# celliern/triflow

Measured on AMD Instinct MI355X. Metric: implicit time-steps/s, 1e6-node 3-var system (member-steps/s over all GPUs), higher is better.
Workload: dtype f64; 1 GPU; BASELINE config 3: M3_film, N=1000000 nodes, periodic, fixed dt=0.001, ROS2; members_per_gpu=1, parallelism=ensemble members sharded by rank, no data-path collective

## Files before the change

__graft_entry__.py:

```python
import os
import sys

ROOT = os.path.dirname(os.path.abspath(__file__))
if ROOT not in sys.path:
    sys.path.insert(0, ROOT)

PREBUILT = ["M1_advdiff", "M2_diff", "M3_film", "M5_stiff"]
PREBUILT_DENSE = ["M3_film", "M5_stiff"]


def build():
    from triflow_amd import compilers, workloads
    from triflow_amd.model import Model
    compilers.build_runtime_library()
    for name in PREBUILT:
        model = Model(*workloads.model_args(name), hold_compilation=True)
        for seg in (4, 8):
            compilers.build_code_object(model, 0, seg=seg)
    saved = os.environ.get("TRIFLOW_BLOCK_MASK")
    os.environ["TRIFLOW_BLOCK_MASK"] = "0"
    try:
        for name in PREBUILT_DENSE:
            model = Model(*workloads.model_args(name), hold_compilation=True)
            compilers.build_code_object(model, 0, seg=4)
    finally:
        if saved is None:
            del os.environ["TRIFLOW_BLOCK_MASK"]
        else:
            os.environ["TRIFLOW_BLOCK_MASK"] = saved
    import triflow_amd


def smoke():
    import numpy as np
    from triflow_amd import Model, schemes, workloads
    from oracle import numpy_path as ora
    name, fd, pars, dt, _ = workloads.config_inputs(3, 4096)
    model = Model(*workloads.model_args(name))
    ref = Model(*workloads.model_args(name), compiler=ora.numpy_compiler)
    F = model.F(model.fields_template(**fd), pars)
    Fo = ref.F(ref.fields_template(**fd), pars)
    assert np.array_equal(F, Fo), "F differs from the oracle"
    J = model.J(model.fields_template(**fd), pars)
    Jo = ref.J(ref.fields_template(**fd), pars)
    assert abs(J - Jo).max() <= 4 * np.spacing(abs(Jo).max()), "J differs from the oracle"
    _, new = schemes.ROS2(model)(0.0, model.fields_template(**fd), dt, pars)
    _, new_o = ora.ROS2(ref)(0.0, ref.fields_template(**fd), dt, pars)
    err = np.abs(new.uflat - new_o.uflat).max() / np.abs(new_o.uflat).max()
    assert err < 1e-9, "ROS2 step differs from the oracle: %g" % err
    print("smoke ok: F bit-exact, J <= 4 ulp, ROS2 step rel err %.1e on %s (N=4096)" % (err, name))


if __name__ == "__main__":
    build()
```

triflow_amd/compilers.py:

```python

import fcntl
import json
import logging
import os
import re
import shutil
import subprocess
import threading
import warnings

import numpy as np
import scipy.sparse as sps

from . import codegen
from ._capi import DeviceModel, DeviceSolver, Library

log = logging.getLogger(__name__)
log.addHandler(logging.NullHandler())

PKG_DIR = os.path.dirname(os.path.abspath(__file__))
CSRC = os.path.join(PKG_DIR, "csrc")
LIB_PATH = os.path.join(PKG_DIR, "lib", "libtriflow_hip.so")
CACHE_DIR = os.path.join(PKG_DIR, "_cache")
GPU_ARCH = "gfx950"
HIPCC_FLAGS = [*os.environ.get("TRIFLOW_HIPCC_OPT", "-O3").split(), "-std=c++17",
               "-ffp-contract=off", "--offload-arch=" + GPU_ARCH,
               *os.environ.get("TRIFLOW_HIPCC_EXTRA", "").split()]

RUNTIME_SOURCES = ("tf_rt_plan.cpp", "tf_rt_io.cpp", "tf_rt_steps.cpp", "tf_rt_diag.cpp",
                   "tf_solver_sweeps.cpp", "tf_solver_linear.cpp", "tf_rt_probe.cpp", "tf_rt_record.cpp",
                   "tf_rt_stat.cpp", "tf_rt_spectrum.cpp", "tf_rt_extrema.cpp")
_SKELETON = ("tf_args.h", "tf_math.h", "tf_kernels.h", "tf_crs.h", "tf_coop_hip.h", "tf_cr2_hip.h", "tf_cr3_hip.h",
             "tf_node.h", "tf_probe.h", "tf_record.h", "tf_stat.h", "tf_spectrum.h", "tf_extrema.h",
             "tf_entry_hip.h")
_TU_HEAD = ('#include <hip/hip_runtime.h>\n'
            '#define TF_DEVICE __device__ __forceinline__\n'
            '%s'
            '#include "tf_math.h"\n')

_TU_TAIL = '#include "tf_kernels.h"\n#include "tf_entry_hip.h"\n'


def _hipcc():
    exe = shutil.which("hipcc") or "/opt/rocm/bin/hipcc"
    if not os.path.exists(exe):
        raise RuntimeError("hipcc not found: the HIP compiler plugin needs the ROCm toolchain")
    return exe


def _skeleton_stamp():
    parts = []
    for name in _SKELETON:
        with open(os.path.join(CSRC, name), "rb") as f:
            parts.append(f.read())
    return codegen.source_hash(*parts)


def build_runtime_library(force=False):
    srcs = [os.path.join(CSRC, n) for n in RUNTIME_SOURCES] + [os.path.join(CSRC, "tf_backend_hip.cpp")]
    deps = srcs + [os.path.join(CSRC, n) for n in ("tf_args.h", "tf_backend.h", "tf_solver.h")] + \
        [os.path.join(os.path.dirname(PKG_DIR), "include", "triflow_hip.h")]
    if not force and os.path.exists(LIB_PATH) and \
            all(os.path.getmtime(LIB_PATH) >= os.path.getmtime(d) for d in deps):
        return LIB_PATH
    os.makedirs(os.path.dirname(LIB_PATH), exist_ok=True)
    cmd = [_hipcc(), "-O2", "-std=c++17", "-fPIC", "-shared", "--offload-arch=" + GPU_ARCH,
           "-I", CSRC, *srcs, "-lpthread", "-o", LIB_PATH + ".tmp"]
    res = subprocess.run(cmd, capture_output=True, text=True)
    if res.returncode != 0:
        raise RuntimeError("building libtriflow_hip.so failed:\n" + res.stderr[-4000:])
    os.replace(LIB_PATH + ".tmp", LIB_PATH)
    return LIB_PATH


def _parse_resource_usage(stderr):
    usage, name = {}, None
    for line in stderr.splitlines():
        m = re.search(r"Function Name: (\S+)", line)
        if m:
            name = m.group(1)
            usage[name] = {}
            continue
        for key, pat in (("VGPRs", r" VGPRs: (\d+)"), ("SGPRs", r" SGPRs: (\d+)"),
                         ("ScratchSize", r"ScratchSize \[bytes/lane\]: (\d+)"),
                         ("Occupancy", r"Occupancy \[waves/SIMD\]: (\d+)")):
            m = re.search(pat, line)
            if m and name:
                usage[name][key] = int(m.group(1))
    return usage


def resource_usage(hsaco_path):
    with open(hsaco_path[:-len(".hsaco")] + ".json") as f:
        return json.load(f)["kernels"]


def _compile_code_object(model, source, tag, hsaco, observer=None):
    global BUILD_COUNT
    BUILD_COUNT += 1
    hip = os.path.join(CACHE_DIR, "model_%s.hip" % tag)
    hip_tmp = hip + ".%d.tmp" % os.getpid()
    with open(hip_tmp, "w") as f:
        f.write(source)
    os.replace(hip_tmp, hip)
    tmp = hsaco + ".%d.tmp" % os.getpid()
    log.info("hipcc: compiling stencil + solver kernels for %s", model._diff_eqs)

    def compile_with(flags, out):
        cmd = [_hipcc(), *flags, "-I", CSRC, "--genco", "--no-gpu-bundle-output",
               "-Rpass-analysis=kernel-resource-usage", "-o", out, hip]
        res = subprocess.run(cmd, capture_output=True, text=True)
        if res.returncode != 0:
            raise RuntimeError("hipcc failed on the generated kernels (%s):\n%s"
                               % (hip, res.stderr[-4000:]))
        return _parse_resource_usage(res.stderr)

    flags = list(HIPCC_FLAGS)
    usage = compile_with(flags, tmp)
    spilled = sorted(k for k, u in usage.items() if u.get("ScratchSize", 0) > 0)
    if observer:
        spilled = [k for k in spilled if k.startswith("tfk_" + observer)]
        if spilled:
            os.remove(tmp)
            raise codegen.UnsupportedExpression(
                "the %s kernels (%s) need more registers than a wavefront has: "
                "use fewer or simpler %ss" % (observer, ", ".join(spilled),
                                               {"stat": "statistic"}.get(observer, observer)))
    alt_flags, alt_usage = None, None
    alt = hsaco[:-len(".hsaco")] + ".alt.hsaco"
    if spilled and "-O1" not in flags and "-O0" not in flags \
            and os.environ.get("TRIFLOW_ALLOW_SCRATCH") != "1":
        _warn_wide(model, spilled)
        alt_flags = ["-O1"] + [f for f in flags if not f.startswith("-O")]
        if os.environ.get("TRIFLOW_SPILL_GATE") == "object":
            flags, alt_flags = alt_flags, None
            usage = compile_with(flags, tmp)
        else:
            alt_usage = compile_with(alt_flags, alt + ".%d.tmp" % os.getpid())
            os.replace(alt + ".%d.tmp" % os.getpid(), alt)
    meta = os.path.join(CACHE_DIR, "model_%s.json" % tag)
    with open(meta + ".%d.tmp" % os.getpid(), "w") as f:
        json.dump(dict(equations=list(model._diff_eqs), flags=flags, kernels=usage,
                       alt_flags=alt_flags, alt_kernels=spilled if alt_flags else [],
                       alt_usage={k: alt_usage[k] for k in spilled} if alt_usage else {},
                       skeleton=_skeleton_stamp(), hipcc=hipcc_version()), f, indent=1)
    os.replace(meta + ".%d.tmp" % os.getpid(), meta)
    os.replace(tmp, hsaco)
    evict_stale_cache()


_warned_wide = set()


def _warn_wide(model, kernels):
    key = tuple(str(e) for e in model._diff_eqs)
    if key in _warned_wide:
        return
    _warned_wide.add(key)
    warnings.warn("triflow_amd: %d kernel(s) of the model %s need more registers than a wavefront has "
                  "(%s spill to scratch): those kernels are built at -O1 and run slower than the "
                  "narrow-model path (DESIGN.md, solver limits)"
                  % (len(kernels), list(key), ", ".join(kernels)), RuntimeWarning, stacklevel=4)


def alternate_of(hsaco_path):
    try:
        with open(hsaco_path[:-len(".hsaco")] + ".json") as f:
            meta = json.load(f)
    except (OSError, ValueError):
        return None, []
    alt = hsaco_path[:-len(".hsaco")] + ".alt.hsaco"
    kernels = meta.get("alt_kernels") or []
    return (alt, kernels) if kernels and os.path.exists(alt) else (None, [])


def _build_locked(model, source, tag, hsaco, observer=None):
    if os.path.exists(hsaco):
        return
    lock_path = hsaco + ".lock"
    try:
        with open(lock_path, "w") as lock:
            try:
                fcntl.flock(lock, fcntl.LOCK_EX)
            except OSError:
                pass
            try:
                if not os.path.exists(hsaco):
                    _compile_code_object(model, source, tag, hsaco, observer)
            finally:
                try:
                    fcntl.flock(lock, fcntl.LOCK_UN)
                except OSError:
                    pass
    finally:
        for leftover in [lock_path] + [os.path.join(CACHE_DIR, n) for n in os.listdir(CACHE_DIR)
                                        if n.endswith(".%d.tmp" % os.getpid())]:
            try:
                os.remove(leftover)
            except OSError:
                pass


def code_object_source(model, parvec_mask=0, seg=8, sweep_block=256):
    body, spec = codegen.lower_model(model, parvec_mask=parvec_mask, seg=seg,
                                     sweep_block=sweep_block)
    source = _TU_HEAD % "" + body + _TU_TAIL
    tag = codegen.source_hash(source, _skeleton_stamp(), " ".join(HIPCC_FLAGS), hipcc_version(), os.environ.get("TRIFLOW_SPILL_GATE", "kernel"), "elf")
    return source, tag, spec


def build_code_object(model, parvec_mask=0, seg=None, sweep_block=None):
    seg = seg or int(os.environ.get("TRIFLOW_SWEEP_SEG", "8"))
    sweep_block = sweep_block or int(os.environ.get("TRIFLOW_SWEEP_BLOCK", "256"))
    source, tag, spec = code_object_source(model, parvec_mask, seg, sweep_block)
    os.makedirs(CACHE_DIR, exist_ok=True)
    hsaco = os.path.join(CACHE_DIR, "model_%s.hsaco" % tag)
    _build_locked(model, source, tag, hsaco)
    return hsaco, spec


def build_observer_code_object(model, block, kind, parvec_mask=0, seg=8, sweep_block=256):
    if kind not in ("probe", "record", "stat", "spectrum", "extrema"):
        raise ValueError("unknown kind of observer %r" % (kind,))
    body, _ = codegen.lower_model(model, parvec_mask=parvec_mask, seg=seg, sweep_block=sweep_block)
    source = _TU_HEAD % "" + body + block + _TU_TAIL
    tag = codegen.source_hash(source, _skeleton_stamp(), " ".join(HIPCC_FLAGS), hipcc_version(), kind, "elf")
    os.makedirs(CACHE_DIR, exist_ok=True)
    hsaco = os.path.join(CACHE_DIR, "model_%s.hsaco" % tag)
    _build_locked(model, source, tag, hsaco, observer=kind)
    return hsaco


_hipcc_version = None
BUILD_COUNT = 0


def hipcc_version():
    global _hipcc_version
    if _hipcc_version is None:
        try:
            res = subprocess.run([_hipcc(), "--version"], capture_output=True, text=True)
            lines = [ln.strip() for ln in res.stdout.splitlines() if ln.strip()]
            _hipcc_version = " / ".join(ln for ln in lines if "version" in ln.lower())[:200] or "unknown"
        except OSError:
            _hipcc_version = "unknown"
    return _hipcc_version


def evict_stale_cache(keep=()):
    if not os.path.isdir(CACHE_DIR):
        return 0
    stamp, ver, removed = _skeleton_stamp(), hipcc_version(), 0
    for name in os.listdir(CACHE_DIR):
        if not (name.startswith("model_") and name.endswith(".json")):
            continue
        base = os.path.join(CACHE_DIR, name[:-len(".json")])
        try:
            with open(base + ".json") as f:
                meta = json.load(f)
        except (OSError, ValueError):
            continue
        if meta.get("skeleton") == stamp and meta.get("hipcc") == ver:
            continue
        if os.path.basename(base) in keep:
            continue
        for ext in (".hsaco", ".alt.hsaco", ".hip", ".json"):
            try:
                os.remove(base + ext)
                removed += 1
            except OSError:
                pass
    return removed


class HipBackend:

    _lib = None
    _lock = threading.Lock()

    def library(self):
        with HipBackend._lock:
            if HipBackend._lib is None:
                HipBackend._lib = Library(LIB_PATH)
            return HipBackend._lib

    def load(self, model, parvec_mask, device=-1, seg=None):
        hsaco, spec = build_code_object(model, parvec_mask, seg=seg)
        lib = self.library()
        is_dev, ndev = lib.runtime_info()
        if ndev < 1:
            raise RuntimeError("no HIP device visible: the triflow_amd compute path needs "
                               "an MI355X (gfx950); there is no CPU fallback")
        if device >= 0:
            lib.set_device(device)
        with open(hsaco, "rb") as f:
            code = f.read()
        alt, alt_kernels = alternate_of(hsaco)
        alt_code = None
        if alt_kernels:
            _warn_wide(model, alt_kernels)
        if alt:
            with open(alt, "rb") as f:
                alt_code = f.read()
        return DeviceModel(lib, spec, code, alt_code, alt_kernels)


_default_backend = HipBackend()


class CscPattern:

    def __init__(self, nvar, mp, sparse_indices, N, periodic):
        k = np.asarray(sparse_indices, dtype=np.int64)
        eq, slot = k % nvar, k // nvar
        var, off = slot % nvar, slot // nvar - mp
        node = np.arange(N, dtype=np.int64)[:, None]
        neigh = node + off[None, :]
        neigh = neigh % N if periodic else np.clip(neigh, 0, N - 1)
        rows = (node * nvar + eq[None, :]).ravel()
        cols = (neigh * nvar + var[None, :]).ravel()
        n = N * nvar
        key = cols * n + rows
        uniq, inverse = np.unique(key, return_inverse=True)
        self.shape = (n, n)
        self.slot = inverse
        self.nslots = uniq.size
        self.indices = (uniq % n).astype(np.int32 if n < 2 ** 31 else np.int64)
        ucols = uniq // n
        self.indptr = np.searchsorted(ucols, np.arange(n + 1)).astype(self.indices.dtype)
        order = np.argsort(inverse, kind="stable")
        first = np.ones(order.size, dtype=bool)
        first[1:] = inverse[order[1:]] != inverse[order[:-1]]
        self.extra_src = order[~first]
        self.extra_slot = inverse[self.extra_src]
        self.gather = np.concatenate([order[first], self.extra_src]).astype(np.int32) \
            if key.size < 2 ** 31 else None

    def assemble(self, values):
        data = np.bincount(self.slot, weights=np.asarray(values).ravel(),
                           minlength=self.nslots)
        return sps.csc_matrix((data, self.indices, self.indptr), shape=self.shape)

    def from_gathered(self, gathered):
        data = gathered[:self.nslots]
        if self.extra_src.size:
            data = data.copy()
            np.add.at(data, self.extra_slot, gathered[self.nslots:])
        return sps.csc_matrix((data, self.indices, self.indptr), shape=self.shape)


class CompiledModel:

    def __init__(self, model, backend=None):
        self.model = model
        self.backend = backend or _default_backend
        self.nvar = model._nvar
        self.fields = list(model._dep_vars) + list(model._help_funcs)
        self.nh = len(model._help_funcs)
        self.pars = list(model._pars)
        self.mp = max((model._window_range - 1) // 2, 1)
        self.real_mp = (model._window_range - 1) // 2
        self._device_models = {}
        self._solvers = {}
        self._patterns = {}
        codegen.lower_model(model)

    @staticmethod
    def sweep_segment(total_nodes):
        if "TRIFLOW_SWEEP_SEG" in os.environ:
            return int(os.environ["TRIFLOW_SWEEP_SEG"])
        return 4 if total_nodes <= 2_000_000 else 8

    def device_model(self, parvec_mask=0, device=-1, seg=None):
        key = (parvec_mask, device, seg)
        if key not in self._device_models:
            kw = {}
            if device >= 0:
                kw["device"] = device
            if seg is not None:
                kw["seg"] = seg
            self._device_models[key] = self.backend.load(self.model, parvec_mask, **kw)
        return self._device_models[key]

    def solver(self, N, periodic, nsys=1, parvec_mask=0, **opts):
        key = (int(N), bool(periodic), int(nsys), int(parvec_mask), tuple(sorted(opts.items())))
        if key not in self._solvers:
            seg = self.sweep_segment(int(N) * int(nsys)) if isinstance(self.backend, HipBackend) else None
            dm = self.device_model(parvec_mask, int(opts.get("device", -1)), seg)
            self._solvers[key] = DeviceSolver(dm, N, nsys=nsys, periodic=periodic, **opts)
        return self._solvers[key]

    def pattern(self, N, periodic):
        key = (int(N), bool(periodic))
        if key not in self._patterns:
            self._patterns[key] = CscPattern(self.nvar, self.real_mp,
                                             self.model._sparse_indices[0], N, periodic)
        return self._patterns[key]

    def release(self):
        for s in self._solvers.values():
            s.close()
        self._solvers.clear()

    @staticmethod
    def grid_spacing(x):
        x = np.asarray(x)
        return (x[-1] - x[0]) / (x.size - 1)

    def parvec_mask_of(self, par_values):
        mask = 0
        for k, v in enumerate(par_values):
            if np.ndim(v) > 0 and np.size(v) > 1 and np.ptp(v) != 0:
                mask |= 1 << k
        return mask

    def bind_inputs(self, solver, x, par_values, helper_arrays=None):
        spec = solver.model.spec
        dx = self.grid_spacing(x)
        solver.set_dx(dx)
        solver.set_x(x)
        mask = spec["parvec_mask"]
        for k, v in enumerate(par_values):
            if (mask >> k) & 1:
                solver.set_param(k, np.asarray(v, dtype=float))
            else:
                solver.set_param(k, float(np.ravel(v)[0]))
        for j, value in enumerate(codegen.eval_host_constants(spec, dx, par_values)):
            solver.set_param(spec["npar_model"] + j, value)
        if self.nh and helper_arrays is not None:
            solver.set_helpers(np.asarray(helper_arrays, dtype=float))

    def _unpack(self, args):
        x = np.asarray(args[0], dtype=float)
        nf = self.nvar + self.nh
        fields = [np.asarray(a, dtype=float) for a in args[1:1 + nf]]
        pars = list(args[1 + nf:1 + nf + len(self.pars)])
        periodic = bool(args[1 + nf + len(self.pars)])
        if len(args) != 2 + nf + len(self.pars):
            raise TypeError("expected %d positional arguments, got %d"
                            % (2 + nf + len(self.pars), len(args)))
        return x, fields, pars, periodic

    def _evaluate(self, args, with_j):
        x, fields, pars, periodic = self._unpack(args)
        mask = self.parvec_mask_of(pars)
        solver = self.solver(x.size, periodic, 1, mask)
        self.bind_inputs(solver, x, pars, fields[self.nvar:] if self.nh else None)
        solver.set_state(0, np.asarray(fields[:self.nvar]))
        solver.eval(0, with_j=with_j)
        return solver, x.size, periodic

    def F_function(self, *args):
        solver, N, periodic = self._evaluate(args, with_j=False)
        return solver.get_F()[0]

    def J_function(self, *args):
        solver, N, periodic = self._evaluate(args, with_j=True)
        pat = self.pattern(N, periodic)
        if pat.gather is None:
            return pat.assemble(solver.get_J()[0])
        if getattr(solver, "_csc_pattern", None) is not pat:
            solver.set_csc_map(pat.gather)
            solver._csc_pattern = pat
        return pat.from_gathered(solver.get_J_mapped())


def hip_compiler(model, backend=None, heaviside=None):
    if heaviside is not None:
        codegen.validate_heaviside(heaviside)
        if getattr(model, "_heaviside", heaviside) != heaviside:
            raise ValueError("heaviside=%r: the model was built with heaviside=%r"
                             % (heaviside, model._heaviside))
        model._heaviside = heaviside
    compiled = CompiledModel(model, backend)

    def F_function(*args):
        return compiled.F_function(*args)

    def J_function(*args):
        return compiled.J_function(*args)

    F_function.device_model = compiled
    J_function.device_model = compiled
    return F_function, J_function


def resolve_compiler(name):
    if name in ("hip", "theano", "numpy"):
        if name != "hip":
            log.info("compiler=%r requested: using the HIP compiler (only back end)", name)
        return hip_compiler
    raise ValueError("unknown compiler %r" % (name,))
```

triflow_amd/csrc/tf_cr3_hip.h:

```cpp
#pragma once

template <int BB> struct TfCr3 {
    static constexpr int MAXLEN = TF_CR_MAXLEN, NPOS = MAXLEN + 1;
    static constexpr int oL = 0, oDL = BB, oU = 2 * BB, oYL = 3 * BB, oDR = 3 * BB + 1, oYR = 4 * BB + 1,
                         oZ = 4 * BB + 2;
    static constexpr int RS = (4 * BB + 3) | 1;
    static constexpr int PS = BB * RS;
    static constexpr int NC = 4 * BB + 1;
    static constexpr bool DUP = NC <= 32;
    static_assert(NC <= 64, "a wavefront holds the augmented columns");
};

__device__ __forceinline__ void tf_st_u(double* ubase, unsigned off8, double v) {
    *(double*)((char*)ubase + off8) = v;
}

template <int BB, int K>
__device__ __forceinline__ void tf_gj3_step(double (&val)[BB], int c, bool& grow) {
    constexpr int PL = BB + K;
    const double pv = tf_readlane_f64(val[K], PL);
    const double rp = tf_rcp_newton(pv);
    if constexpr (K + 1 < BB) {
        double mx = 0.0;
#pragma unroll
        for (int i = K + 1; i < BB; ++i) mx = __builtin_fmax(mx, tf_abs(val[i]));
        if (c == PL && !(mx <= TF_GJ_GROWTH * tf_abs(val[K]))) grow = true;
    }
    const double pr = val[K] * rp;
#pragma unroll
    for (int i = 0; i < BB; ++i) {
        if (i == K) continue;
        const double m = tf_readlane_f64(val[i], PL);
        val[i] = tf_fma(-m, pr, val[i]);
    }
    val[K] = pr;
    if constexpr (K + 1 < BB) tf_gj3_step<BB, K + 1>(val, c, grow);
}

template <int BB>
__device__ __forceinline__ void tfk_cr_factor_v4(const TfLevelArgs& a) {
    typedef TfCr3<BB> C;
    constexpr int NPOS = C::NPOS, B2 = BB * BB, REC = 4 * B2, NT_MIN = 256;
    constexpr int RS = C::RS, PS = C::PS, NC = C::NC;
    constexpr int oL = C::oL, oDL = C::oDL, oU = C::oU, oYL = C::oYL, oDR = C::oDR, oYR = C::oYR, oZ = C::oZ;
    constexpr int NO = 2 * BB + 1;
    constexpr int NQ = (2 * B2 + 63) / 64;
    const int NT = blockDim.x, nw = NT >> 6;
    const TfLayout& L = a.L;
    const TfCrChunk<BB> ch(L, (int)blockIdx.x);
    const int tid = threadIdx.x, w = __builtin_amdgcn_readfirstlane(tid >> 6), lane = tid & 63;
    constexpr bool DUP = C::DUP;
    const int half = DUP ? lane >> 5 : 0, c = DUP ? lane & 31 : lane;
    const int mI = ch.mI, pe = ch.pe, len = ch.len;
    const bool with_rhs = a.cr_rhs != 0;

    __shared__ double sRow[NPOS * PS];
    __shared__ unsigned sPerm[NPOS + 1];
    auto row = [&](int pos, int r) { return sRow + pos * PS + r * RS; };
    unsigned* const perm = a.perm + ch.nbase + ch.start;
    if (tid < len) sPerm[tid + 1] = perm[tid];
    unsigned* const perm_top = a.perm + (int64_t)L.nsys * L.N + ch.e;
    if (a.fold_top && tid == 64) sPerm[0] = *perm_top;

    const bool cL = c < BB, cD = c >= BB && c < 2 * BB, cU = c >= 2 * BB && c < 3 * BB, cY = c == 3 * BB,
               cI = c > 3 * BB && c < NC;
    const int off1 = cL ? oL + c : (cD ? oDL + c - BB : (cU ? oU + c - 2 * BB : (cY ? oYL : oZ)));
    const int off2 = cD ? oDR + c - BB : (cY ? oYR : oZ);
    const int idc = cI ? c - 3 * BB - 1 : -1;
    const bool keepE = half == 0 && (cL || cU), keepZ = half == 0 && cY;
    const bool grec = half == 0 && (cL || cU || cI);
    const unsigned goff = (unsigned)((cI ? idc : (cL ? B2 + c : 2 * B2 + c - 2 * BB)) * 8);
    const bool pvalid = cL || cU || cY;
    auto pacc_of = [&](int sd) { return sd == 0 ? (cL || cY) : (cU || cY); };
    auto pslot_of = [&](int sd) { return sd == 0 ? (cL ? oDR + c : (cU ? oU + c - 2 * BB : oYR))
                                                 : (cL ? oL + c : (cU ? oDL + c - 2 * BB : oYL)); };
    const int pslot0 = pslot_of(DUP ? half : 0), pslot1 = pslot_of(1);
    const bool pacc0 = pacc_of(DUP ? half : 0), pacc1 = pacc_of(1);
    const int opoff0 = (DUP ? half : 0) ? oL : oU;
    int crel[NQ];
    bool cside[NQ], cok[NQ];
#pragma unroll
    for (int q = 0; q < NQ; ++q) {
        const int e = lane + 64 * q, sd = e >= B2 ? 1 : 0, j = e - sd * B2;
        cok[q] = e < 2 * B2;
        cside[q] = sd != 0;
        crel[q] = cok[q] ? (j / BB) * RS + (sd ? oL : oU) + j % BB : 0;
    }

    TF_STAMP_REAL(a, 30);
    TF_STAMP(a, 0);
    {
        const double* src = a.Ablk + (ch.nbase + ch.start) * REC;
        const int n3 = len * 3 * B2;
        constexpr int NIT = (C::MAXLEN * 3 * B2 + NT_MIN - 1) / NT_MIN;
        double v[NIT], v2[NIT];
#pragma unroll
        for (int it = 0; it < NIT; ++it) {
            const int i = it * NT + tid;
            const int nd = i / (3 * B2), rem = i - nd * 3 * B2, blk = rem / B2, rc = rem - blk * B2;
            v[it] = i < n3 ? src[nd * REC + blk * B2 + rc] : 0.0;
            v2[it] = (i < n3 && blk == 1) ? src[nd * REC + 3 * B2 + rc] : 0.0;
        }
        const double* prev = a.Ablk + (ch.nbase + ch.gprev) * REC + 2 * B2;
        double p0 = 0.0, y0 = 0.0;
        if (tid < B2 && ch.has_prev) p0 = prev[tid];
        const double* ys = a.rhs + (ch.nbase + ch.start) * 2 * BB;
        if (with_rhs && tid < len * BB) y0 = ys[(tid / BB) * 2 * BB + tid % BB] + ys[(tid / BB) * 2 * BB + BB + tid % BB];
        for (int i = tid; i < (len + 1) * BB * (RS - 3 * BB); i += NT) {
            const int pr = i / (RS - 3 * BB), o = i - pr * (RS - 3 * BB);
            sRow[(pr / BB) * PS + (pr % BB) * RS + 3 * BB + o] = 0.0;
        }
        if (tid < 3 * B2) {
            const int blk = tid / B2, rc = tid - blk * B2, r = rc / BB, cc = rc - r * BB;
            row(0, r)[blk * BB + cc] = 0.0;
        }
#pragma unroll
        for (int it = 0; it < NIT; ++it) {
            const int i = it * NT + tid;
            const int nd = i / (3 * B2), rem = i - nd * 3 * B2, blk = rem / B2, rc = rem - blk * B2;
            const int r = rc / BB, cc = rc - r * BB;
            if (i < n3) row(nd + 1, r)[blk * BB + cc] = v[it] + v2[it];
        }
        __syncthreads();
        if (tid < B2) row(0, tid / BB)[oU + tid % BB] = p0;
        if (tid < len * BB) row(tid / BB + 1, tid % BB)[oYL] = y0;
        if (!L.periodic) {
            if (ch.start == 0 && tid < B2) row(1, tid / BB)[oL + tid % BB] = 0.0;
            if (ch.start + len == L.N && tid >= 64 && tid < 64 + B2) row(pe, (tid - 64) / BB)[oU + (tid - 64) % BB] = 0.0;
        }
    }
    __syncthreads();

    bool ok = true;
    TF_STAMP(a, 1);
    int stamp_i = 2;
    for (int r = 0; (1 << r) <= mI; ++r) {
        const int s = 1 << r;
        const int nA = ((mI >> r) + 1) >> 1;
        for (int t = w; t < nA; t += nw) {
            const int k = s * (2 * t + 1);
            const int ia = k - s, ib = k + s <= mI ? k + s : pe;
            const double* rk = row(k, 0);
            double* ra = row(ia, 0);
            double* rb = row(ib, 0);
            double* nb = (DUP && half) ? rb : ra;
            if (r == 1) TF_STAMP(a, 44);
            double old[BB], old1[DUP ? 1 : BB], cp[NQ];
#pragma unroll
            for (int i = 0; i < BB; ++i) old[i] = nb[i * RS + pslot0];
            if constexpr (!DUP) {
#pragma unroll
                for (int i = 0; i < BB; ++i) old1[i] = rb[i * RS + pslot1];
            }
#pragma unroll
            for (int q = 0; q < NQ; ++q) cp[q] = (cside[q] ? rb : ra)[crel[q]];
            unsigned code = (unsigned)__builtin_amdgcn_readfirstlane((int)sPerm[k]);
            double val[BB];
            bool done = false;
#pragma unroll 1
            for (int attempt = 0; attempt < 2 && !done; ++attempt) {
#pragma unroll
                for (int i = 0; i < BB; ++i) {
                    const int src = (int)(((code >> (3 * i)) & 7u) ^ (unsigned)i);
                    const double* rr = rk + src * RS;
                    const double v = rr[off1] + rr[off2];
                    val[i] = idc == src ? 1.0 : v;
                }
                bool grow = false;
                tf_gj3_step<BB, 0>(val, c, grow);
                double chk = 0.0;
#pragma unroll
                for (int i = 0; i < BB; ++i) chk += val[i] - val[i];
                if (c < NC && !(chk == 0.0)) grow = true;
                done = __builtin_amdgcn_ballot_w64(grow) == 0ull;
                TF_COUNT(a, 41);
                if (!done) {
                    if (attempt == 1) { ok = false; break; }
                    TF_COUNT(a, 40);
                    constexpr int NJ = (NC + 7) / 8;
                    const int g = lane & 7, h = lane >> 3;
                    double sv[NJ];
#pragma unroll
                    for (int j = 0; j < NJ; ++j) {
                        const int cc = h + 8 * j;
                        const double* rr = rk + (g < BB ? g : 0) * RS;
                        double v = 0.0;
                        if (g < BB) {
                            if (cc < BB) v = rr[oL + cc];
                            else if (cc < 2 * BB) v = rr[oDL + cc - BB] + rr[oDR + cc - BB];
                            else if (cc < 3 * BB) v = rr[oU + cc - 2 * BB];
                            else if (cc == 3 * BB) v = rr[oYL] + rr[oYR];
                            else if (cc < NC) v = cc - 3 * BB - 1 == g ? 1.0 : 0.0;
                        }
                        sv[j] = v;
                    }
                    const int myk = tf_gj_wave<BB, NC, BB>(sv, g, h, ok);
                    unsigned bits = 0;
                    if (g < BB && h == 0) {
                        if (myk >= 0) bits = ((unsigned)(g ^ myk)) << (3 * myk); else ok = false;
                    }
                    code = (unsigned)__builtin_amdgcn_readfirstlane((int)tf_group8_or(bits));
                    if (lane == 0) perm[k - 1] = code;
                }
            }
            if (r == 1) TF_STAMP(a, 45);
            {
                double* rec = a.crf + (ch.nbase + ch.node(k)) * 5 * B2;
                if (grec) {
#pragma unroll
                    for (int i = 0; i < BB; ++i) tf_st_u(rec, goff + (unsigned)(i * BB * 8), val[i]);
                }
#pragma unroll
                for (int q = 0; q < NQ; ++q)
                    if (cok[q]) tf_st_u(rec, (unsigned)((3 * B2 + lane + 64 * q) * 8), cp[q]);
                double* rkw = row(k, 0);
                if (keepZ || (keepE && a.fold_top)) {
#pragma unroll
                    for (int i = 0; i < BB; ++i) rkw[i * RS + off1] = val[i];
                }
            }
            if (r == 1) TF_STAMP(a, 46);
            auto update = [&](double* nbp, int opoff, int pslot, bool pacc, const double* oldv) {
                const double* opb = nbp + opoff;
                double out[BB];
#pragma unroll
                for (int i = 0; i < BB; ++i) {
                    double acc = 0.0;
#pragma unroll
                    for (int m = 0; m < BB; ++m) acc = tf_fma(-opb[i * RS + m], val[m], acc);
                    out[i] = acc;
                }
                if (pvalid) {
#pragma unroll
                    for (int i = 0; i < BB; ++i) nbp[i * RS + pslot] = (pacc ? oldv[i] : 0.0) + out[i];
                }
            };
            update(nb, opoff0, pslot0, pacc0, old);
            if (r == 1) TF_STAMP(a, 47);
            if constexpr (!DUP) update(rb, oL, pslot1, pacc1, old1);
            if (r == 1) TF_STAMP(a, 48);
        }
        TF_STAMP(a, stamp_i); ++stamp_i;
        __syncthreads();
        TF_STAMP(a, stamp_i); ++stamp_i;
    }

    if (with_rhs) {
        double* zt = a.zt + (ch.nbase + ch.start) * BB;
        for (int i = tid; i < mI * BB; i += NT) zt[i] = row(i / BB + 1, i % BB)[oYL];
    }
    for (int i = tid; i < 2 * BB * NO; i += NT) {
        const int side = i / (BB * NO), rem = i - side * BB * NO, r = rem / NO, o = rem - r * NO;
        const int nn = side == 0 ? ch.p : ch.pprev;
        double* rec = a.Anext + ((int64_t)ch.e * a.Lnext.N + nn) * REC;
        double* rr = a.rhsnext + ((int64_t)ch.e * a.Lnext.N + nn) * 2 * BB;
        const double* rs = row(side == 0 ? pe : 0, r);
        if (o < BB) rec[(side == 0 ? 0 : 2) * B2 + r * BB + o] = rs[(side == 0 ? oL : oU) + o];
        else if (o < 2 * BB) rec[(side == 0 ? 1 : 3) * B2 + r * BB + o - BB] = rs[oDL + o - BB] + rs[oDR + o - BB];
        else if (with_rhs) rr[(side == 0 ? 0 : BB) + r] = rs[oYL] + rs[oYR];
    }
    TF_STAMP(a, 20);
    if (a.fold_top) {
        __syncthreads();
        constexpr int NCT = 2 * BB + 1, NJT = (NCT + 7) / 8;
        const int g = lane & 7, h = lane >> 3;
        if (w == 0) {
            const double* r0 = row(0, 0);
            const double* rp = row(pe, 0);
            double val[NJT];
            unsigned code = sPerm[0];
            const unsigned code0 = code;
            const int myk = tf_gj_node<BB, NCT, 0>(val, g, h, code, ok, [&](int rr, int cc) {
                const int o = rr * RS;
                return rr < 0 ? 0.0 : (cc < BB ? rp[o + oL + cc] + (rp[o + oDL + cc] + rp[o + oDR + cc]) + r0[o + oU + cc]
                                                     + (r0[o + oDL + cc] + r0[o + oDR + cc])
                       : (cc == BB ? (rp[o + oYL] + rp[o + oYR]) + (r0[o + oYL] + r0[o + oYR])
                                   : ((cc < NCT && cc - BB - 1 == rr) ? 1.0 : 0.0))); });
            if (code != code0 && lane == 0) *perm_top = code;
            if (g < BB) {
                const int nsys = L.Ptot;
#pragma unroll
                for (int j = 0; j < NJT; ++j) {
                    const int cc = h + 8 * j;
                    if (cc > BB && cc < NCT) a.topAinv[(int64_t)(myk * BB + cc - BB - 1) * nsys + ch.e] = val[j];
                    if (cc == BB && with_rhs) {
                        const double x = val[j];
                        a.topx[(int64_t)ch.e * BB + myk] = x;
                        a.x[(ch.nbase + ch.node(pe)) * BB + myk] = x;
                        row(pe, myk)[oYL] = x;
                        row(0, myk)[oYL] = ch.has_prev ? x : 0.0;
                    }
                }
            }
        }
        if (with_rhs) {
            __syncthreads();
            int r = 0;
            while ((2 << r) <= mI) ++r;
            for (; r >= 0; --r) {
                const int s = 1 << r;
                const int nA = ((mI >> r) + 1) >> 1;
                for (int t = w; t < nA; t += nw) {
                    if (!(h == 0 && g < BB)) continue;
                    const int k = s * (2 * t + 1);
                    const int kl = k - s, kr = k + s <= mI ? k + s : pe;
                    double* rk = row(k, g);
                    double xk = rk[oYL];
#pragma unroll
                    for (int m = 0; m < BB; ++m) {
                        xk = tf_fma(-rk[oL + m], row(kl, m)[oYL], xk);
                        xk = tf_fma(-rk[oU + m], row(kr, m)[oYL], xk);
                    }
                    rk[oYL] = xk;
                    a.x[(ch.nbase + ch.node(k)) * BB + g] = xk;
                }
                __syncthreads();
            }
        }
    }
    if (!ok && lane == 0) *a.status = 1;
    TF_STAMP(a, 21);
    TF_STAMP_REAL(a, 31);
}
```

Measured before the change: 2668 steps/s.

## Use wide double2 loads and stores for cyclic-reduction block I/O

Adds a wide-I/O path to the 3-block cyclic reduction kernel. Node blocks are loaded as double2 pairs, reduced-system blocks are written out as double2, and factor records are staged through LDS so each wavefront stores them contiguously. The goal is fewer, coalesced global memory transactions, at the cost of extra LDS traffic, a wave sync and more complex index mapping. The path is on by default, and a narrow fallback build is kept via a macro.

```diff
diff --git a/__graft_entry__.py b/__graft_entry__.py
--- a/__graft_entry__.py
+++ b/__graft_entry__.py
@@ -7,6 +7,7 @@
 
 PREBUILT = ["M1_advdiff", "M2_diff", "M3_film", "M5_stiff"]
 PREBUILT_DENSE = ["M3_film", "M5_stiff"]
+PREBUILT_CR_NARROW = ["M3_film", "M5_stiff", "tri3", "wide4"]
 
 
 def build():
@@ -28,6 +29,13 @@
             del os.environ["TRIFLOW_BLOCK_MASK"]
         else:
             os.environ["TRIFLOW_BLOCK_MASK"] = saved
+    from oracle import corpus
+    for name in PREBUILT_CR_NARROW:
+        model = Model(*corpus.model_args(name), hold_compilation=True)
+        if name not in PREBUILT:
+            compilers.build_code_object(model, 0, seg=4)
+        with compilers.extra_flags("-DTF_CR_WIDE_IO=0"):
+            compilers.build_code_object(model, 0, seg=4)
     import triflow_amd
 
 
diff --git a/triflow_amd/compilers.py b/triflow_amd/compilers.py
--- a/triflow_amd/compilers.py
+++ b/triflow_amd/compilers.py
@@ -1,4 +1,5 @@
 
+import contextlib
 import fcntl
 import json
 import logging
@@ -27,10 +28,22 @@
                "-ffp-contract=off", "--offload-arch=" + GPU_ARCH,
                *os.environ.get("TRIFLOW_HIPCC_EXTRA", "").split()]
 
+
+@contextlib.contextmanager
+def extra_flags(*flags):
+    saved = list(HIPCC_FLAGS)
+    HIPCC_FLAGS.extend(flags)
+    try:
+        yield
+    finally:
+        HIPCC_FLAGS[:] = saved
+
+
 RUNTIME_SOURCES = ("tf_rt_plan.cpp", "tf_rt_io.cpp", "tf_rt_steps.cpp", "tf_rt_diag.cpp",
                    "tf_solver_sweeps.cpp", "tf_solver_linear.cpp", "tf_rt_probe.cpp", "tf_rt_record.cpp",
                    "tf_rt_stat.cpp", "tf_rt_spectrum.cpp", "tf_rt_extrema.cpp")
 _SKELETON = ("tf_args.h", "tf_math.h", "tf_kernels.h", "tf_crs.h", "tf_coop_hip.h", "tf_cr2_hip.h", "tf_cr3_hip.h",
+             "tf_cr_io.h",
              "tf_node.h", "tf_probe.h", "tf_record.h", "tf_stat.h", "tf_spectrum.h", "tf_extrema.h",
              "tf_entry_hip.h")
 _TU_HEAD = ('#include <hip/hip_runtime.h>\n'
diff --git a/triflow_amd/csrc/tf_cr3_hip.h b/triflow_amd/csrc/tf_cr3_hip.h
--- a/triflow_amd/csrc/tf_cr3_hip.h
+++ b/triflow_amd/csrc/tf_cr3_hip.h
@@ -1,4 +1,18 @@
 #pragma once
+#include "tf_cr_io.h"
+
+#ifndef TF_CR_WIDE_IO
+#define TF_CR_WIDE_IO 1
+#endif
+#ifndef TF_CR_WIDE_LOAD
+#define TF_CR_WIDE_LOAD TF_CR_WIDE_IO
+#endif
+#ifndef TF_CR_WIDE_SHARE
+#define TF_CR_WIDE_SHARE TF_CR_WIDE_IO
+#endif
+#ifndef TF_CR_WIDE_REC
+#define TF_CR_WIDE_REC TF_CR_WIDE_IO
+#endif
 
 template <int BB> struct TfCr3 {
     static constexpr int MAXLEN = TF_CR_MAXLEN, NPOS = MAXLEN + 1;
@@ -9,6 +23,9 @@
     static constexpr int NC = 4 * BB + 1;
     static constexpr bool DUP = NC <= 32;
     static_assert(NC <= 64, "a wavefront holds the augmented columns");
+    typedef TfCrWide<BB> Io;
+    static_assert(Io::RS == RS && Io::PS == PS && Io::oL == oL && Io::oDL == oDL && Io::oU == oU && Io::oYL == oYL &&
+                  Io::oDR == oDR && Io::oYR == oYR, "tf_cr_io.h describes this row layout");
 };
 
 __device__ __forceinline__ void tf_st_u(double* ubase, unsigned off8, double v) {
@@ -87,15 +104,45 @@
         crel[q] = cok[q] ? (j / BB) * RS + (sd ? oL : oU) + j % BB : 0;
     }
 
+    typedef typename C::Io Io;
+    constexpr int NQ3 = (3 * B2 + 63) / 64;
+    const bool stage = half == 0 && c < NC && !cD;
+    const int soff = cI ? oDR + idc : off1;
+    int srel[NQ3];
+    bool sok[NQ3];
+    if constexpr (TF_CR_WIDE_REC) {
+#pragma unroll
+        for (int q = 0; q < NQ3; ++q) {
+            const int e = lane + 64 * q;
+            sok[q] = e < 3 * B2;
+            srel[q] = sok[q] ? Io::record_slot(e) : 0;
+        }
+    }
+
     TF_STAMP_REAL(a, 30);
     TF_STAMP(a, 0);
     {
         const double* src = a.Ablk + (ch.nbase + ch.start) * REC;
+        constexpr int NITW = (C::MAXLEN + NT_MIN / B2 - 1) / (NT_MIN / B2);
+        int ndl, wq;
+        bool wact;
+        Io::thread(tid, NT, ndl, wq, wact);
+        const int npi = __builtin_amdgcn_readfirstlane(Io::nodes_per_pass(NT));
+        double2 va[TF_CR_WIDE_LOAD ? NITW : 1], vb[TF_CR_WIDE_LOAD ? NITW : 1];
+        if constexpr (TF_CR_WIDE_LOAD) {
+#pragma unroll
+            for (int it = 0; it < NITW; ++it) {
+                const int nd = ndl + it * npi, ndc = nd < len ? nd : len - 1;
+                const char* p = (const char*)src + (unsigned)((ndc * REC + 2 * wq) * 8);
+                va[it] = *(const double2*)p;
+                vb[it] = *(const double2*)(p + 2 * B2 * 8);
+            }
+        }
         const int n3 = len * 3 * B2;
         constexpr int NIT = (C::MAXLEN * 3 * B2 + NT_MIN - 1) / NT_MIN;
-        double v[NIT], v2[NIT];
-#pragma unroll
-        for (int it = 0; it < NIT; ++it) {
+        double v[TF_CR_WIDE_LOAD ? 1 : NIT], v2[TF_CR_WIDE_LOAD ? 1 : NIT];
+#pragma unroll
+        for (int it = 0; it < (TF_CR_WIDE_LOAD ? 0 : NIT); ++it) {
             const int i = it * NT + tid;
             const int nd = i / (3 * B2), rem = i - nd * 3 * B2, blk = rem / B2, rc = rem - blk * B2;
             v[it] = i < n3 ? src[nd * REC + blk * B2 + rc] : 0.0;
@@ -106,20 +153,46 @@
         if (tid < B2 && ch.has_prev) p0 = prev[tid];
         const double* ys = a.rhs + (ch.nbase + ch.start) * 2 * BB;
         if (with_rhs && tid < len * BB) y0 = ys[(tid / BB) * 2 * BB + tid % BB] + ys[(tid / BB) * 2 * BB + BB + tid % BB];
-        for (int i = tid; i < (len + 1) * BB * (RS - 3 * BB); i += NT) {
-            const int pr = i / (RS - 3 * BB), o = i - pr * (RS - 3 * BB);
-            sRow[(pr / BB) * PS + (pr % BB) * RS + 3 * BB + o] = 0.0;
-        }
-        if (tid < 3 * B2) {
-            const int blk = tid / B2, rc = tid - blk * B2, r = rc / BB, cc = rc - r * BB;
-            row(0, r)[blk * BB + cc] = 0.0;
-        }
-#pragma unroll
-        for (int it = 0; it < NIT; ++it) {
-            const int i = it * NT + tid;
-            const int nd = i / (3 * B2), rem = i - nd * 3 * B2, blk = rem / B2, rc = rem - blk * B2;
-            const int r = rc / BB, cc = rc - r * BB;
-            if (i < n3) row(nd + 1, r)[blk * BB + cc] = v[it] + v2[it];
+        if constexpr (TF_CR_WIDE_LOAD) {
+            for (int i = tid; i < PS; i += NT) sRow[i] = 0.0;
+            int ws[2], wz[Io::NZ];
+            bool wd[2];
+            Io::pair(wq, 0, ws[0], wd[0]);
+            Io::pair(wq, 1, ws[1], wd[1]);
+#pragma unroll
+            for (int j = 0; j < Io::NZ; ++j) wz[j] = Io::zero_slot(wq, j);
+#pragma unroll
+            for (int it = 0; it < NITW; ++it) {
+                const int nd = ndl + it * npi;
+                double* pos = sRow + (nd + 1) * PS;
+                if (wact && nd < len) {
+#pragma unroll
+                    for (int h = 0; h < 2; ++h) {
+                        const double x = h ? va[it].y : va[it].x, y = h ? vb[it].y : vb[it].x;
+                        pos[ws[h]] = x + (wd[h] ? y : 0.0);
+                        if (!wd[h]) pos[ws[h] + 2 * BB] = y + 0.0;
+                    }
+#pragma unroll
+                    for (int j = 0; j < Io::NZ; ++j)
+                        if (wz[j] >= 0) pos[wz[j]] = 0.0;
+                }
+            }
+        } else {
+            for (int i = tid; i < (len + 1) * BB * (RS - 3 * BB); i += NT) {
+                const int pr = i / (RS - 3 * BB), o = i - pr * (RS - 3 * BB);
+                sRow[(pr / BB) * PS + (pr % BB) * RS + 3 * BB + o] = 0.0;
+            }
+            if (tid < 3 * B2) {
+                const int blk = tid / B2, rc = tid - blk * B2, r = rc / BB, cc = rc - r * BB;
+                row(0, r)[blk * BB + cc] = 0.0;
+            }
+#pragma unroll
+            for (int it = 0; it < NIT; ++it) {
+                const int i = it * NT + tid;
+                const int nd = i / (3 * B2), rem = i - nd * 3 * B2, blk = rem / B2, rc = rem - blk * B2;
+                const int r = rc / BB, cc = rc - r * BB;
+                if (i < n3) row(nd + 1, r)[blk * BB + cc] = v[it] + v2[it];
+            }
         }
         __syncthreads();
         if (tid < B2) row(0, tid / BB)[oU + tid % BB] = p0;
@@ -206,15 +279,27 @@
             if (r == 1) TF_STAMP(a, 45);
             {
                 double* rec = a.crf + (ch.nbase + ch.node(k)) * 5 * B2;
-                if (grec) {
+                double* rkw = row(k, 0);
+                if constexpr (TF_CR_WIDE_REC) {
+                    if (stage) {
+#pragma unroll
+                        for (int i = 0; i < BB; ++i) rkw[i * RS + soff] = val[i];
+                    }
+                    TF_WAVE_SYNC();
+                    double sv[NQ3];
+#pragma unroll
+                    for (int q = 0; q < NQ3; ++q) sv[q] = rkw[srel[q]];
+#pragma unroll
+                    for (int q = 0; q < NQ3; ++q)
+                        if (sok[q]) tf_st_u(rec, (unsigned)((lane + 64 * q) * 8), sv[q]);
+                } else if (grec) {
 #pragma unroll
                     for (int i = 0; i < BB; ++i) tf_st_u(rec, goff + (unsigned)(i * BB * 8), val[i]);
                 }
 #pragma unroll
                 for (int q = 0; q < NQ; ++q)
                     if (cok[q]) tf_st_u(rec, (unsigned)((3 * B2 + lane + 64 * q) * 8), cp[q]);
-                double* rkw = row(k, 0);
-                if (keepZ || (keepE && a.fold_top)) {
+                if (!TF_CR_WIDE_REC && (keepZ || (keepE && a.fold_top))) {
 #pragma unroll
                     for (int i = 0; i < BB; ++i) rkw[i * RS + off1] = val[i];
                 }
@@ -249,15 +334,44 @@
         double* zt = a.zt + (ch.nbase + ch.start) * BB;
         for (int i = tid; i < mI * BB; i += NT) zt[i] = row(i / BB + 1, i % BB)[oYL];
     }
-    for (int i = tid; i < 2 * BB * NO; i += NT) {
-        const int side = i / (BB * NO), rem = i - side * BB * NO, r = rem / NO, o = rem - r * NO;
-        const int nn = side == 0 ? ch.p : ch.pprev;
-        double* rec = a.Anext + ((int64_t)ch.e * a.Lnext.N + nn) * REC;
-        double* rr = a.rhsnext + ((int64_t)ch.e * a.Lnext.N + nn) * 2 * BB;
-        const double* rs = row(side == 0 ? pe : 0, r);
-        if (o < BB) rec[(side == 0 ? 0 : 2) * B2 + r * BB + o] = rs[(side == 0 ? oL : oU) + o];
-        else if (o < 2 * BB) rec[(side == 0 ? 1 : 3) * B2 + r * BB + o - BB] = rs[oDL + o - BB] + rs[oDR + o - BB];
-        else if (with_rhs) rr[(side == 0 ? 0 : BB) + r] = rs[oYL] + rs[oYR];
+    if constexpr (TF_CR_WIDE_SHARE) {
+        int side, q, rside, rr_r;
+        bool act, ract;
+        Io::share_thread(tid, side, q, act);
+        Io::share_rhs_thread(tid, rside, rr_r, ract);
+        if (act) {
+            const int nn = side == 0 ? ch.p : ch.pprev;
+            double* rec = a.Anext + ((int64_t)ch.e * a.Lnext.N + nn) * REC + side * 2 * B2;
+            const double* rs = row(side == 0 ? pe : 0, 0) + side * 2 * BB;
+            double o[2];
+#pragma unroll
+            for (int h = 0; h < 2; ++h) {
+                int slot;
+                bool dia;
+                Io::pair(q, h, slot, dia);
+                const double* ps = dia ? rs - side * 2 * BB + slot : rs + slot;
+                const double x = ps[0], y = ps[dia ? oDR - oDL : 0];
+                o[h] = dia ? x + y : x;
+            }
+            *(double2*)(rec + 2 * q) = make_double2(o[0], o[1]);
+        }
+        if (ract && with_rhs) {
+            const int nn = rside == 0 ? ch.p : ch.pprev;
+            double* rr = a.rhsnext + ((int64_t)ch.e * a.Lnext.N + nn) * 2 * BB;
+            const double* rs = row(rside == 0 ? pe : 0, rr_r);
+            rr[(rside == 0 ? 0 : BB) + rr_r] = rs[oYL] + rs[oYR];
+        }
+    } else {
+        for (int i = tid; i < 2 * BB * NO; i += NT) {
+            const int side = i / (BB * NO), rem = i - side * BB * NO, r = rem / NO, o = rem - r * NO;
+            const int nn = side == 0 ? ch.p : ch.pprev;
+            double* rec = a.Anext + ((int64_t)ch.e * a.Lnext.N + nn) * REC;
+            double* rr = a.rhsnext + ((int64_t)ch.e * a.Lnext.N + nn) * 2 * BB;
+            const double* rs = row(side == 0 ? pe : 0, r);
+            if (o < BB) rec[(side == 0 ? 0 : 2) * B2 + r * BB + o] = rs[(side == 0 ? oL : oU) + o];
+            else if (o < 2 * BB) rec[(side == 0 ? 1 : 3) * B2 + r * BB + o - BB] = rs[oDL + o - BB] + rs[oDR + o - BB];
+            else if (with_rhs) rr[(side == 0 ? 0 : BB) + r] = rs[oYL] + rs[oYR];
+        }
     }
     TF_STAMP(a, 20);
     if (a.fold_top) {
diff --git a/triflow_amd/csrc/tf_cr_io.h b/triflow_amd/csrc/tf_cr_io.h
--- /dev/null
+++ b/triflow_amd/csrc/tf_cr_io.h
@@ -0,0 +1,43 @@
+#pragma once
+
+#if defined(__HIPCC__)
+#define TF_CRIO_FN __host__ __device__ __forceinline__
+#else
+#define TF_CRIO_FN inline
+#endif
+
+template <int BB> struct TfCrWide {
+    static constexpr int B2 = BB * BB, REC = 4 * B2;
+    static constexpr int oL = 0, oDL = BB, oU = 2 * BB, oYL = 3 * BB, oDR = 3 * BB + 1, oYR = 4 * BB + 1;
+    static constexpr int RS = (4 * BB + 3) | 1, PS = BB * RS;
+    static constexpr int ZW = RS - 3 * BB, NZS = BB * ZW, NZ = (NZS + B2 - 1) / B2;
+
+    static TF_CRIO_FN int nodes_per_pass(int nt) { return nt / B2; }
+    static TF_CRIO_FN void thread(int tid, int nt, int& ndl, int& q, bool& active) {
+        ndl = tid / B2; q = tid - ndl * B2; active = ndl < nodes_per_pass(nt);
+    }
+    static TF_CRIO_FN void pair(int q, int h, int& slot, bool& dia) {
+        const int e = 2 * q + h;
+        dia = e >= B2;
+        const int rc = dia ? e - B2 : e, r = rc / BB, cc = rc - r * BB;
+        slot = r * RS + (dia ? oDL : oL) + cc;
+    }
+    static TF_CRIO_FN int zero_slot(int q, int j) {
+        const int z = q + j * B2;
+        if (z >= NZS) return -1;
+        const int r = z / ZW;
+        return r * RS + 3 * BB + (z - r * ZW);
+    }
+    static constexpr int SH = (B2 + 63) & ~63;
+    static TF_CRIO_FN void share_thread(int tid, int& side, int& q, bool& active) {
+        side = tid >= SH ? 1 : 0; q = tid - side * SH; active = q >= 0 && q < B2;
+    }
+    static TF_CRIO_FN void share_rhs_thread(int tid, int& side, int& r, bool& active) {
+        const int t = tid - 2 * SH;
+        side = t >= BB ? 1 : 0; r = t - side * BB; active = t >= 0 && t < 2 * BB;
+    }
+    static TF_CRIO_FN int record_slot(int e) {
+        const int blk = e / B2, rc = e - blk * B2, i = rc / BB, cc = rc - i * BB;
+        return i * RS + (blk == 0 ? oDR : (blk == 1 ? oL : oU)) + cc;
+    }
+};
```

Measured after the change: 2702 steps/s (median of 6 runs). 1.01x the previous value.
